# ELEKTRONN/ELEKTRONN2

Hardware: AMD Instinct MI355X
Metric: training_input_voxels_per_sec (higher is better)
Workload: dtype f32; 1 GPU; neuro3d_lite (1,1,23,183,183)->(1,2,10,37,37) fwd+bwd+Adam, 1 sample/GPU; parallelism=dp1, hipgraph=True, steps_per_launch=10

## Files before the change

elektronn2_amd/csrc/conv_first_mfma.hip:

```cpp
#include "common.hpp"
#include <algorithm>
#include <utility>

typedef float f32x4 __attribute__((ext_vector_type(4)));

template <class F, int... I>
__device__ __forceinline__ void fm_for_impl(F&& f, std::integer_sequence<int, I...>) {
  (f(std::integral_constant<int, I>{}), ...);
}
template <int N, class F>
__device__ __forceinline__ void fm_for(F&& f) {
  fm_for_impl(f, std::make_integer_sequence<int, N>{});
}
template <int ABID>
__device__ __forceinline__ f32x4 fm_mfma(float a, float b, f32x4 c) {
  return __builtin_amdgcn_mfma_f32_4x4x1f32(a, b, c, 4, ABID, 0);
}

namespace {

typedef __bf16 fm_bf16x8 __attribute__((ext_vector_type(8)));

struct FirstM {
  const float* x;
  const float* w;
  const float* bias;
  float* out;
  const float* dout;
  int N, Cout, D, H, W;
  int Ho, Wo;
  long xsN, xsD, xsH;
  long osN, osC, osD, osH;
  int act;
  int tilesX, tilesY, nTiles;
  int dbg;
  __bf16* nxb;
  int nxKG;
};

#ifdef E2_DEBUG_ENV
#define FM_DBG(p, bit) (((p).dbg & (bit)) != 0)
#else
#define FM_DBG(p, bit) false
#endif

constexpr int kTW = 72;

template <int KH, int KW, int PY, int PX, int MG>
struct Geo {
  static constexpr int T = KH * KW;
  static constexpr int TPV = 16 / MG;
  static constexpr int NAV = (T + TPV - 1) / TPV;
  static constexpr int RT = 4 * PY + KH - 1;
  static constexpr int CH = 4 * MG;
};

template <int KH, int KW, int PY, int PX, int MG>
__device__ __forceinline__ void load_weights(const FirstM& p, int lane,
                                             float (&aw)[Geo<KH, KW, PY, PX, MG>::NAV]) {
  using G = Geo<KH, KW, PY, PX, MG>;
  const int b = lane >> 2, i = lane & 3;
  const int slot = b / MG, g = b - slot * MG;
  const int ch = 4 * g + i;
#pragma unroll
  for (int v = 0; v < G::NAV; ++v) {
    const int tap = v * G::TPV + slot;
    aw[v] = (slot < G::TPV && tap < G::T && ch < p.Cout) ? p.w[ch * G::T + (G::T - 1 - tap)] : 0.f;
  }
}

template <int KH, int KW, int PY, int PX, int MG>
__device__ __forceinline__ void load_tile(const FirstM& p, int tile, float* xt, int& n, int& z,
                                          int& row0, int& col0) {
  using G = Geo<KH, KW, PY, PX, MG>;
  const int tx_ = tile % p.tilesX;
  int r = tile / p.tilesX;
  const int ty_ = r % p.tilesY; r /= p.tilesY;
  z = r % p.D;
  n = r / p.D;
  row0 = ty_ * 4 * PY;
  col0 = tx_ * 64;
  const float* src = p.x + (long)n * p.xsN + (long)z * p.xsD;
  for (int e = threadIdx.x; e < G::RT * kTW; e += 256) {
    const int i = e / kTW, j = e - i * kTW;
    const int y = row0 + i, xx = col0 + j;
    xt[e] = (y < p.H && xx < p.W && !FM_DBG(p, 1)) ? src[(long)y * p.xsH + xx] : 0.f;
  }
}

template <int KH, int KW, int PY, int PX, int MG>
__device__ __forceinline__ void conv_rows(const float* xw, int lane,
                                          const float (&aw)[Geo<KH, KW, PY, PX, MG>::NAV],
                                          f32x4 (&acc)[MG][PY]) {
  using G = Geo<KH, KW, PY, PX, MG>;
#pragma unroll
  for (int g = 0; g < MG; ++g)
#pragma unroll
    for (int nb = 0; nb < PY; ++nb) acc[g][nb] = (f32x4){0.f, 0.f, 0.f, 0.f};
  fm_for<PY + KH - 1>([&](auto rr_) {
    constexpr int rr = decltype(rr_)::value;
    float bx[KW];
#pragma unroll
    for (int tx = 0; tx < KW; ++tx) bx[tx] = xw[rr * kTW + lane + tx];
    fm_for<PY>([&](auto nb_) {
      constexpr int nb = decltype(nb_)::value;
      constexpr int ty = rr - nb;
      if constexpr (ty >= 0 && ty < KH) {
        fm_for<KW>([&](auto tx_) {
          constexpr int tx = decltype(tx_)::value;
          constexpr int tap = ty * KW + tx;
          fm_for<MG>([&](auto g_) {
            constexpr int g = decltype(g_)::value;
            acc[g][nb] = fm_mfma<(tap % G::TPV) * MG + g>(aw[tap / G::TPV], bx[tx], acc[g][nb]);
          });
        });
      }
    });
  });
}

template <int KH, int KW, int PY, int PX, int MG>
__global__ __launch_bounds__(256) void firstm_fwd_kernel(FirstM p) {
  using G = Geo<KH, KW, PY, PX, MG>;
  __shared__ float xt[G::RT * kTW];
  const int lane = threadIdx.x & 63, wave = threadIdx.x >> 6;
  float aw[G::NAV];
  load_weights<KH, KW, PY, PX, MG>(p, lane, aw);
  float bs[MG][4];
#pragma unroll
  for (int g = 0; g < MG; ++g)
#pragma unroll
    for (int r = 0; r < 4; ++r) bs[g][r] = (4 * g + r < p.Cout) ? p.bias[4 * g + r] : 0.f;
  for (int tile = blockIdx.x; tile < p.nTiles; tile += gridDim.x) {
    int n, z, row0, col0;
    __syncthreads();
    load_tile<KH, KW, PY, PX, MG>(p, tile, xt, n, z, row0, col0);
    __syncthreads();
    f32x4 acc[MG][PY];
    if (!FM_DBG(p, 2)) conv_rows<KH, KW, PY, PX, MG>(xt + wave * PY * kTW, lane, aw, acc);
    else {
#pragma unroll
      for (int g = 0; g < MG; ++g)
#pragma unroll
        for (int nb = 0; nb < PY; ++nb) acc[g][nb] = (f32x4){xt[lane], 0.f, 0.f, 0.f};
    }
    const int prow = row0 / PY + wave;
    const int pcol = (col0 + lane) / PX;
    const bool ok = prow < p.Ho && pcol < p.Wo && (lane % PX) == 0;
    float* ob = p.out + (long)n * p.osN + (long)z * p.osD + (long)prow * p.osH + pcol;
#pragma unroll
    for (int g = 0; g < MG; ++g)
#pragma unroll
      for (int r = 0; r < 4; ++r) {
        float m = acc[g][0][r];
        if constexpr (PY == 2) m = fmaxf(m, acc[g][1][r]);
        if constexpr (PX == 2) m = fmaxf(m, __shfl_xor(m, 1, 64));
        const int ch = 4 * g + r;
        float v = 0.f;
        if (ch < p.Cout) {
          v = m + bs[g][r];
          if (p.act == E2_ACT_RELU) v = fmaxf(v, 0.f);
          if (ok && !(FM_DBG(p, 4) && ch > 0)) ob[(long)ch * p.osC] = v;
        }
        acc[g][0][r] = v;
      }
    if (p.nxb && ok) {
      __bf16* nb = p.nxb + ((((long)n * p.D + z) * p.nxKG) * ((long)p.Ho * p.Wo) + (long)prow * p.Wo + pcol) * 8;
#pragma unroll
      for (int kg = 0; kg < (MG + 1) / 2; ++kg) {
        if (kg >= p.nxKG) continue;
        fm_bf16x8 h;
#pragma unroll
        for (int e = 0; e < 8; ++e) {
          const int g = 2 * kg + (e >> 2);
          h[e] = (__bf16)(g < MG ? acc[g < MG ? g : 0][0][e & 3] : 0.f);
        }
        *reinterpret_cast<fm_bf16x8*>(nb + (long)kg * p.Ho * p.Wo * 8) = h;
      }
    }
  }
}

template <int KH, int KW, int PY, int PX, int MG>
__global__ __launch_bounds__(256) void firstm_bwd_kernel(FirstM p, float* __restrict__ part) {
  using G = Geo<KH, KW, PY, PX, MG>;
  constexpr int T = G::T, CH = G::CH, NP = 64 * PY;
  constexpr bool Q4 = T <= 16;
  extern __shared__ __attribute__((aligned(16))) float fm_lds[];
  float* dyT = fm_lds;
  float* xt = fm_lds + 4 * NP * CH;
  const int lane = threadIdx.x & 63, wave = threadIdx.x >> 6;
  float aw[G::NAV];
  load_weights<KH, KW, PY, PX, MG>(p, lane, aw);
  const int pq = Q4 ? (lane >> 4) : 0;
  const int tapi = Q4 ? (lane & 15) : lane;
  const int tapl = tapi < T ? tapi : 0;
  const int tapoff = (tapl / KW) * kTW + (tapl % KW) + pq;
  f32x4 dwacc[MG];
  float db[MG][4];
#pragma unroll
  for (int g = 0; g < MG; ++g) {
    dwacc[g] = (f32x4){0.f, 0.f, 0.f, 0.f};
#pragma unroll
    for (int r = 0; r < 4; ++r) db[g][r] = 0.f;
  }
  float* dyw = dyT + wave * NP * CH;
  float bs[MG][4];
#pragma unroll
  for (int g = 0; g < MG; ++g)
#pragma unroll
    for (int r = 0; r < 4; ++r) bs[g][r] = (4 * g + r < p.Cout) ? p.bias[4 * g + r] : 0.f;
  for (int tile = blockIdx.x; tile < p.nTiles; tile += gridDim.x) {
    int n, z, row0, col0;
    __syncthreads();
    load_tile<KH, KW, PY, PX, MG>(p, tile, xt, n, z, row0, col0);
    const int prow = row0 / PY + wave;
    const int pcol = (col0 + lane) / PX;
    const bool ok = prow < p.Ho && pcol < p.Wo;
    const float* gp = p.dout + (long)n * p.osN + (long)z * p.osD + (long)prow * p.osH + pcol;
    float gvs[MG][4];
#pragma unroll
    for (int g = 0; g < MG; ++g)
#pragma unroll
      for (int r = 0; r < 4; ++r)
        gvs[g][r] = (ok && 4 * g + r < p.Cout) ? gp[(long)(4 * g + r) * p.osC] : 0.f;
    __syncthreads();
    const float* xw = xt + wave * PY * kTW;
    f32x4 acc[MG][PY];
    if (!FM_DBG(p, 2)) conv_rows<KH, KW, PY, PX, MG>(xw, lane, aw, acc);
    else {
#pragma unroll
      for (int g = 0; g < MG; ++g)
#pragma unroll
        for (int nb = 0; nb < PY; ++nb) acc[g][nb] = (f32x4){xw[lane], 0.f, 0.f, 0.f};
    }
#pragma unroll
    for (int g = 0; g < MG; ++g) {
#pragma unroll
      for (int r = 0; r < 4; ++r) {
        float m = acc[g][0][r];
        if constexpr (PY == 2) m = fmaxf(m, acc[g][1][r]);
        if constexpr (PX == 2) m = fmaxf(m, __shfl_xor(m, 1, 64));
        float gv = gvs[g][r];
        if (p.act == E2_ACT_RELU) {
          const float pre = m + bs[g][r];
          gv *= (pre > 0.f) ? 1.f : ((pre == 0.f) ? 0.5f : 0.f);
        }
        if ((lane % PX) == 0) db[g][r] += gv;
#pragma unroll
        for (int nb = 0; nb < PY; ++nb) acc[g][nb][r] = (acc[g][nb][r] == m) ? gv : 0.f;
      }
#pragma unroll
      for (int nb = 0; nb < PY; ++nb)
        *reinterpret_cast<f32x4*>(dyw + (nb * 64 + lane) * CH + 4 * g) = acc[g][nb];
    }
    const float* xb = xw + tapoff;
    if (FM_DBG(p, 4)) continue;
    if constexpr (Q4) {
      fm_for<NP / 4>([&](auto k_) {
        constexpr int p0 = 4 * decltype(k_)::value;
        const float bv = xb[(p0 / 64) * kTW + (p0 % 64)];
#pragma unroll
        for (int g = 0; g < MG; ++g) {
          const float av = dyw[(p0 + pq) * CH + 4 * g + (lane & 3)];
          dwacc[g] = __builtin_amdgcn_mfma_f32_4x4x1f32(av, bv, dwacc[g], 0, 0, 0);
        }
      });
    } else {
      fm_for<NP / 16>([&](auto pb_) {
        constexpr int pb = decltype(pb_)::value;
        float ad[MG];
#pragma unroll
        for (int g = 0; g < MG; ++g) ad[g] = dyw[(pb * 16 + (lane >> 2)) * CH + 4 * g + (lane & 3)];
        fm_for<16>([&](auto pp_) {
          constexpr int pp = decltype(pp_)::value;
          constexpr int pos = pb * 16 + pp;
          const float bv = xb[(pos / 64) * kTW + (pos % 64)];
#pragma unroll
          for (int g = 0; g < MG; ++g) dwacc[g] = fm_mfma<pp>(ad[g], bv, dwacc[g]);
        });
      });
    }
  }
  __syncthreads();
  float* red = fm_lds;
#pragma unroll
  for (int g = 0; g < MG; ++g)
#pragma unroll
    for (int r = 0; r < 4; ++r) {
      float v = dwacc[g][r];
      if constexpr (Q4) {
        v += __shfl_xor(v, 16, 64);
        v += __shfl_xor(v, 32, 64);
      }
      float sb = db[g][r];
#pragma unroll
      for (int o = 32; o > 0; o >>= 1) sb += __shfl_xor(sb, o, 64);
      float* rw = red + (wave * CH + 4 * g + r) * (T + 1);
      if (lane < T) rw[lane] = v;
      if (lane == 0) rw[T] = sb;
    }
  __syncthreads();
  float* ps = part + blockIdx.x;
  const long nS = gridDim.x;
  for (int e = threadIdx.x; e < p.Cout * (T + 1); e += 256)
    ps[e * nS] = (red[e] + red[CH * (T + 1) + e]) + (red[2 * CH * (T + 1) + e] + red[3 * CH * (T + 1) + e]);
}

template <int KH, int KW, int PY, int PX, int MG>
int launch_fwd(e2_ctx* ctx, const FirstM& p, int grid) {
  hipLaunchKernelGGL((firstm_fwd_kernel<KH, KW, PY, PX, MG>), dim3(grid), dim3(256), 0, ctx->stream, p);
  E2_CHECK_HIP(hipGetLastError());
  return 0;
}
template <int KH, int KW, int PY, int PX, int MG>
int launch_bwd(e2_ctx* ctx, const FirstM& p, int grid, float* part) {
  using G = Geo<KH, KW, PY, PX, MG>;
  const size_t lds = sizeof(float) * (4 * 64 * PY * G::CH + G::RT * kTW);
  static bool attr_done = false;
  if (!attr_done) {
    E2_CHECK_HIP(hipFuncSetAttribute(reinterpret_cast<const void*>(&firstm_bwd_kernel<KH, KW, PY, PX, MG>),
                                     hipFuncAttributeMaxDynamicSharedMemorySize, 160 * 1024));
    attr_done = true;
  }
  hipLaunchKernelGGL((firstm_bwd_kernel<KH, KW, PY, PX, MG>), dim3(grid), dim3(256), lds, ctx->stream, p, part);
  E2_CHECK_HIP(hipGetLastError());
  return 0;
}

}

int e2i_firstm_mg(int cout) { return cout <= 20 ? 5 : (cout <= 32 ? 8 : 0); }

int e2i_firstm_grid(const e2_ctx* ctx, long nTiles) {
  return (int)std::min<long>(nTiles, std::min<long>((long)ctx->num_cu * (e2_dbg_env("E2_FM_GRID") ? e2_dbg_env_int("E2_FM_GRID") : 3), 1024));
}

static void fill(FirstM& p, const e2_tensor5* x, const e2_tensor5* o, int cout, int py, int px) {
  p.x = x->ptr;
  p.N = x->n; p.Cout = cout; p.D = x->d; p.H = x->h; p.W = x->w;
  p.Ho = o->h; p.Wo = o->w;
  p.xsN = x->sn; p.xsD = x->sd; p.xsH = x->sh;
  p.osN = o->sn; p.osC = o->sc; p.osD = o->sd; p.osH = o->sh;
  p.dbg = e2_dbg_env_int("E2_FM_DBG");
  p.tilesX = e2_cdiv(o->w * px, 64);
  p.tilesY = e2_cdiv(o->h, 4);
  p.nTiles = p.N * p.D * p.tilesY * p.tilesX;
}

#define E2_FM_DISPATCH(FN, ...)                                                        \
  if (v == 1 && mg == 5) return FN<4, 4, 2, 2, 5>(__VA_ARGS__);                       \
  if (v == 1 && mg == 8) return FN<4, 4, 2, 2, 8>(__VA_ARGS__);                       \
  if (v == 2 && mg == 5) return FN<6, 6, 2, 2, 5>(__VA_ARGS__);                       \
  if (v == 2 && mg == 8) return FN<6, 6, 2, 2, 8>(__VA_ARGS__);                       \
  if (v == 3 && mg == 5) return FN<3, 3, 1, 1, 5>(__VA_ARGS__);                       \
  if (v == 3 && mg == 8) return FN<3, 3, 1, 1, 8>(__VA_ARGS__);

int e2i_firstm_fwd(e2_ctx* ctx, int v, const e2_tensor5* x, const float* w, const float* bias,
                   int cout, int py, int px, int act, const e2_tensor5* out, void* next_xb, int next_kg) {
  const int mg = e2i_firstm_mg(cout);
  FirstM p{};
  fill(p, x, out, cout, py, px);
  p.w = w; p.bias = bias; p.out = out->ptr; p.act = act;
  E2_REQUIRE(!next_xb || (next_kg * 8 >= cout && ((uintptr_t)next_xb & 15) == 0),
             "conv1(mfma): the next layer's copy holds %d channel groups for %d channels", next_kg, cout);
  p.nxb = reinterpret_cast<__bf16*>(next_xb); p.nxKG = next_kg;
  const int grid = e2i_firstm_grid(ctx, p.nTiles);
  E2_FM_DISPATCH(launch_fwd, ctx, p, grid)
  e2_set_error("conv1(mfma): no instance for variant %d, %d channels", v, cout);
  return 2;
}

size_t e2i_firstm_ws_floats(long nTiles, int cout, int T) {
  return (size_t)std::min<long>(nTiles, 1024) * cout * (T + 1);
}

int e2i_firstm_bwd(e2_ctx* ctx, int v, const e2_tensor5* x, const float* w, const float* bias,
                   const e2_tensor5* dout, int py, int px, int act, float* part, int* nslots) {
  const int cout = dout->c;
  const int mg = e2i_firstm_mg(cout);
  FirstM p{};
  fill(p, x, dout, cout, py, px);
  p.w = w; p.bias = bias; p.dout = dout->ptr; p.act = act;
  const int grid = e2i_firstm_grid(ctx, p.nTiles);
  *nslots = grid;
  E2_FM_DISPATCH(launch_bwd, ctx, p, grid, part)
  e2_set_error("conv1(mfma): no instance for variant %d, %d channels", v, cout);
  return 2;
}
```

Measured before the change: 521.9 million voxels/s.

## Trim index math and loads in first-layer MFMA conv kernels

Replaces the per-tile integer div/mod tile decode with precomputed magic-number division and switches strides to 32-bit unsigned offsets, checked on the host. The tile load is restructured from a strided loop into unrolled per-wave row loads with a separate halo load. The max-pool neighbour exchange uses DPP instead of a shuffle, and the epilogue is specialised for relu and full-channel cases. The backward pass folds the activation test into an infinite bias when there is no relu. The aim is to cut scalar and vector integer overhead in a small, latency-bound first layer, at the cost of more code and range checks that reject large tensors.

```diff
diff --git a/elektronn2_amd/csrc/conv_first_mfma.hip b/elektronn2_amd/csrc/conv_first_mfma.hip
--- a/elektronn2_amd/csrc/conv_first_mfma.hip
+++ b/elektronn2_amd/csrc/conv_first_mfma.hip
@@ -17,9 +17,31 @@
   return __builtin_amdgcn_mfma_f32_4x4x1f32(a, b, c, 4, ABID, 0);
 }
 
+__device__ __forceinline__ float fm_xor1(float v) {
+  return __int_as_float(__builtin_amdgcn_mov_dpp(__float_as_int(v), 0xB1, 0xF, 0xF, true));
+}
+
+__device__ __forceinline__ int fm_per_tile(int v) {
+  asm volatile("" : "+s"(v));
+  return v;
+}
+
 namespace {
 
 typedef __bf16 fm_bf16x8 __attribute__((ext_vector_type(8)));
+
+struct FmDiv { unsigned m, sh; };
+inline FmDiv fm_mk_div(unsigned d) {
+  unsigned l = 0;
+  while ((1ull << l) < d) ++l;
+  FmDiv f;
+  f.m = (unsigned)(((1ull << (31 + l)) + d - 1) / d);
+  f.sh = l;
+  return f;
+}
+__device__ __forceinline__ unsigned fm_div(unsigned n, const FmDiv& f) {
+  return __umulhi(2u * n + 1u, f.m) >> f.sh;
+}
 
 struct FirstM {
   const float* x;
@@ -29,10 +51,11 @@
   const float* dout;
   int N, Cout, D, H, W;
   int Ho, Wo;
-  long xsN, xsD, xsH;
-  long osN, osC, osD, osH;
+  unsigned xsN, xsD, xsH;
+  unsigned osN, osC, osD, osH;
   int act;
   int tilesX, tilesY, nTiles;
+  FmDiv dX, dY, dD;
   int dbg;
   __bf16* nxb;
   int nxKG;
@@ -52,6 +75,7 @@
   static constexpr int TPV = 16 / MG;
   static constexpr int NAV = (T + TPV - 1) / TPV;
   static constexpr int RT = 4 * PY + KH - 1;
+  static constexpr int RTL = (RT + 7) / 8 * 8;
   static constexpr int CH = 4 * MG;
 };
 
@@ -69,23 +93,39 @@
   }
 }
 
-template <int KH, int KW, int PY, int PX, int MG>
-__device__ __forceinline__ void load_tile(const FirstM& p, int tile, float* xt, int& n, int& z,
-                                          int& row0, int& col0) {
-  using G = Geo<KH, KW, PY, PX, MG>;
-  const int tx_ = tile % p.tilesX;
-  int r = tile / p.tilesX;
-  const int ty_ = r % p.tilesY; r /= p.tilesY;
-  z = r % p.D;
-  n = r / p.D;
-  row0 = ty_ * 4 * PY;
-  col0 = tx_ * 64;
-  const float* src = p.x + (long)n * p.xsN + (long)z * p.xsD;
-  for (int e = threadIdx.x; e < G::RT * kTW; e += 256) {
-    const int i = e / kTW, j = e - i * kTW;
-    const int y = row0 + i, xx = col0 + j;
-    xt[e] = (y < p.H && xx < p.W && !FM_DBG(p, 1)) ? src[(long)y * p.xsH + xx] : 0.f;
-  }
+template <int PY>
+__device__ __forceinline__ void decode_tile(const FirstM& p, int tile, int& n, int& z, int& row0, int& col0) {
+  const unsigned r1 = fm_div((unsigned)tile, p.dX), tx_ = (unsigned)tile - r1 * (unsigned)p.tilesX;
+  const unsigned r2 = fm_div(r1, p.dY), ty_ = r1 - r2 * (unsigned)p.tilesY;
+  const unsigned n_ = fm_div(r2, p.dD);
+  n = (int)n_;
+  z = (int)(r2 - n_ * (unsigned)p.D);
+  row0 = (int)ty_ * 4 * PY;
+  col0 = (int)tx_ * 64;
+}
+
+template <int KH, int KW, int PY, int PX, int MG>
+__device__ __forceinline__ void load_tile(const FirstM& p, float* xt, int lane, int wave, int n, int z,
+                                          int row0, int col0) {
+  using G = Geo<KH, KW, PY, PX, MG>;
+  const float* src = p.x + (unsigned long)n * p.xsN + (unsigned long)z * p.xsD +
+                     (unsigned long)row0 * p.xsH + col0;
+  const int hrem = p.H - row0, wrem = p.W - col0;
+  float v[G::RTL / 4 + 1];
+  bool in[G::RTL / 4 + 1];
+#pragma unroll
+  for (int k = 0; k < G::RTL / 4; ++k) {
+    const int i = wave + 4 * k;
+    in[k] = i < hrem && lane < wrem && !FM_DBG(p, 1);
+    v[k] = src[in[k] ? (unsigned)i * p.xsH + (unsigned)lane : 0u];
+  }
+  const int hi = 4 * wave + (lane >> 3), hj = 64 + (lane & 7);
+  const bool halo = lane < 32 && hi < G::RTL;
+  in[G::RTL / 4] = halo && hi < hrem && hj < wrem && !FM_DBG(p, 1);
+  v[G::RTL / 4] = src[in[G::RTL / 4] ? (unsigned)hi * p.xsH + (unsigned)hj : 0u];
+#pragma unroll
+  for (int k = 0; k < G::RTL / 4; ++k) xt[(wave + 4 * k) * kTW + lane] = in[k] ? v[k] : 0.f;
+  if (halo) xt[hi * kTW + hj] = in[G::RTL / 4] ? v[G::RTL / 4] : 0.f;
 }
 
 template <int KH, int KW, int PY, int PX, int MG>
@@ -120,10 +160,10 @@
 }
 
 template <int KH, int KW, int PY, int PX, int MG>
-__global__ __launch_bounds__(256) void firstm_fwd_kernel(FirstM p) {
-  using G = Geo<KH, KW, PY, PX, MG>;
-  __shared__ float xt[G::RT * kTW];
-  const int lane = threadIdx.x & 63, wave = threadIdx.x >> 6;
+__global__ __launch_bounds__(256, 3) void firstm_fwd_kernel(FirstM p) {
+  using G = Geo<KH, KW, PY, PX, MG>;
+  __shared__ float xt[G::RTL * kTW];
+  const int lane = threadIdx.x & 63, wave = __builtin_amdgcn_readfirstlane(threadIdx.x >> 6);
   float aw[G::NAV];
   load_weights<KH, KW, PY, PX, MG>(p, lane, aw);
   float bs[MG][4];
@@ -131,10 +171,13 @@
   for (int g = 0; g < MG; ++g)
 #pragma unroll
     for (int r = 0; r < 4; ++r) bs[g][r] = (4 * g + r < p.Cout) ? p.bias[4 * g + r] : 0.f;
+  const bool relu = p.act == E2_ACT_RELU, full = p.Cout == G::CH;
+  const unsigned cstep = p.osC * 4u;
   for (int tile = blockIdx.x; tile < p.nTiles; tile += gridDim.x) {
     int n, z, row0, col0;
+    decode_tile<PY>(p, tile, n, z, row0, col0);
     __syncthreads();
-    load_tile<KH, KW, PY, PX, MG>(p, tile, xt, n, z, row0, col0);
+    load_tile<KH, KW, PY, PX, MG>(p, xt, lane, wave, n, z, row0, col0);
     __syncthreads();
     f32x4 acc[MG][PY];
     if (!FM_DBG(p, 2)) conv_rows<KH, KW, PY, PX, MG>(xt + wave * PY * kTW, lane, aw, acc);
@@ -147,35 +190,64 @@
     const int prow = row0 / PY + wave;
     const int pcol = (col0 + lane) / PX;
     const bool ok = prow < p.Ho && pcol < p.Wo && (lane % PX) == 0;
-    float* ob = p.out + (long)n * p.osN + (long)z * p.osD + (long)prow * p.osH + pcol;
 #pragma unroll
     for (int g = 0; g < MG; ++g)
 #pragma unroll
       for (int r = 0; r < 4; ++r) {
         float m = acc[g][0][r];
         if constexpr (PY == 2) m = fmaxf(m, acc[g][1][r]);
-        if constexpr (PX == 2) m = fmaxf(m, __shfl_xor(m, 1, 64));
-        const int ch = 4 * g + r;
-        float v = 0.f;
-        if (ch < p.Cout) {
-          v = m + bs[g][r];
-          if (p.act == E2_ACT_RELU) v = fmaxf(v, 0.f);
-          if (ok && !(FM_DBG(p, 4) && ch > 0)) ob[(long)ch * p.osC] = v;
+        if constexpr (PX == 2) m = fmaxf(m, fm_xor1(m));
+        acc[g][0][r] = m;
+      }
+    auto epilogue = [&](auto relu_, auto full_) {
+      constexpr bool RELU = decltype(relu_)::value, FULL = decltype(full_)::value;
+      const int cout = FULL ? G::CH : fm_per_tile(p.Cout);
+#pragma unroll
+      for (int g = 0; g < MG; ++g)
+#pragma unroll
+        for (int r = 0; r < 4; ++r) {
+          float v = 0.f;
+          if (FULL || 4 * g + r < cout) {
+            v = acc[g][0][r] + bs[g][r];
+            if constexpr (RELU) v = fmaxf(v, 0.f);
+          }
+          acc[g][0][r] = v;
         }
-        acc[g][0][r] = v;
-      }
-    if (p.nxb && ok) {
-      __bf16* nb = p.nxb + ((((long)n * p.D + z) * p.nxKG) * ((long)p.Ho * p.Wo) + (long)prow * p.Wo + pcol) * 8;
-#pragma unroll
-      for (int kg = 0; kg < (MG + 1) / 2; ++kg) {
-        if (kg >= p.nxKG) continue;
-        fm_bf16x8 h;
-#pragma unroll
-        for (int e = 0; e < 8; ++e) {
-          const int g = 2 * kg + (e >> 2);
-          h[e] = (__bf16)(g < MG ? acc[g < MG ? g : 0][0][e & 3] : 0.f);
+      if (ok) {
+        char* ob = reinterpret_cast<char*>(p.out + (unsigned long)n * p.osN + (unsigned long)z * p.osD);
+        unsigned vo = ((unsigned)prow * p.osH + (unsigned)pcol) * 4u;
+#pragma unroll
+        for (int g = 0; g < MG; ++g)
+#pragma unroll
+          for (int r = 0; r < 4; ++r) {
+            const int ch = 4 * g + r;
+            if ((FULL || ch < cout) && !(FM_DBG(p, 4) && ch > 0)) *reinterpret_cast<float*>(ob + vo) = acc[g][0][r];
+            vo += cstep;
+          }
+      }
+    };
+    if (relu) {
+      if (full) epilogue(std::true_type{}, std::true_type{});
+      else epilogue(std::true_type{}, std::false_type{});
+    } else {
+      if (full) epilogue(std::false_type{}, std::true_type{});
+      else epilogue(std::false_type{}, std::false_type{});
+    }
+    if (p.nxb) {
+      const int nkg = fm_per_tile(p.nxKG);
+      __bf16* nb = p.nxb + ((((long)n * p.D + z) * nkg) * ((long)p.Ho * p.Wo) + (long)prow * p.Wo + pcol) * 8;
+      if (ok) {
+#pragma unroll
+        for (int kg = 0; kg < (MG + 1) / 2; ++kg) {
+          if (kg >= nkg) continue;
+          fm_bf16x8 h;
+#pragma unroll
+          for (int e = 0; e < 8; ++e) {
+            const int g = 2 * kg + (e >> 2);
+            h[e] = (__bf16)(g < MG ? acc[g < MG ? g : 0][0][e & 3] : 0.f);
+          }
+          *reinterpret_cast<fm_bf16x8*>(nb + (long)kg * p.Ho * p.Wo * 8) = h;
         }
-        *reinterpret_cast<fm_bf16x8*>(nb + (long)kg * p.Ho * p.Wo * 8) = h;
       }
     }
   }
@@ -189,7 +261,7 @@
   extern __shared__ __attribute__((aligned(16))) float fm_lds[];
   float* dyT = fm_lds;
   float* xt = fm_lds + 4 * NP * CH;
-  const int lane = threadIdx.x & 63, wave = threadIdx.x >> 6;
+  const int lane = threadIdx.x & 63, wave = __builtin_amdgcn_readfirstlane(threadIdx.x >> 6);
   float aw[G::NAV];
   load_weights<KH, KW, PY, PX, MG>(p, lane, aw);
   const int pq = Q4 ? (lane >> 4) : 0;
@@ -210,20 +282,49 @@
   for (int g = 0; g < MG; ++g)
 #pragma unroll
     for (int r = 0; r < 4; ++r) bs[g][r] = (4 * g + r < p.Cout) ? p.bias[4 * g + r] : 0.f;
+  if (p.act != E2_ACT_RELU) {
+#pragma unroll
+    for (int g = 0; g < MG; ++g)
+#pragma unroll
+      for (int r = 0; r < 4; ++r) bs[g][r] = __builtin_inff();
+  }
+  const bool full = p.Cout == CH;
+  const unsigned cstep = p.osC * 4u;
   for (int tile = blockIdx.x; tile < p.nTiles; tile += gridDim.x) {
     int n, z, row0, col0;
+    decode_tile<PY>(p, tile, n, z, row0, col0);
     __syncthreads();
-    load_tile<KH, KW, PY, PX, MG>(p, tile, xt, n, z, row0, col0);
+    load_tile<KH, KW, PY, PX, MG>(p, xt, lane, wave, n, z, row0, col0);
     const int prow = row0 / PY + wave;
     const int pcol = (col0 + lane) / PX;
     const bool ok = prow < p.Ho && pcol < p.Wo;
-    const float* gp = p.dout + (long)n * p.osN + (long)z * p.osD + (long)prow * p.osH + pcol;
     float gvs[MG][4];
 #pragma unroll
     for (int g = 0; g < MG; ++g)
 #pragma unroll
-      for (int r = 0; r < 4; ++r)
-        gvs[g][r] = (ok && 4 * g + r < p.Cout) ? gp[(long)(4 * g + r) * p.osC] : 0.f;
+      for (int r = 0; r < 4; ++r) gvs[g][r] = 0.f;
+    if (ok) {
+      const char* gb = reinterpret_cast<const char*>(p.dout + (unsigned long)n * p.osN + (unsigned long)z * p.osD);
+      unsigned vo = ((unsigned)prow * p.osH + (unsigned)pcol) * 4u;
+      if (full) {
+#pragma unroll
+        for (int g = 0; g < MG; ++g)
+#pragma unroll
+          for (int r = 0; r < 4; ++r) {
+            gvs[g][r] = *reinterpret_cast<const float*>(gb + vo);
+            vo += cstep;
+          }
+      } else {
+        const int cout = fm_per_tile(p.Cout);
+#pragma unroll
+        for (int g = 0; g < MG; ++g)
+#pragma unroll
+          for (int r = 0; r < 4; ++r) {
+            if (4 * g + r < cout) gvs[g][r] = *reinterpret_cast<const float*>(gb + vo);
+            vo += cstep;
+          }
+      }
+    }
     __syncthreads();
     const float* xw = xt + wave * PY * kTW;
     f32x4 acc[MG][PY];
@@ -240,13 +341,11 @@
       for (int r = 0; r < 4; ++r) {
         float m = acc[g][0][r];
         if constexpr (PY == 2) m = fmaxf(m, acc[g][1][r]);
-        if constexpr (PX == 2) m = fmaxf(m, __shfl_xor(m, 1, 64));
+        if constexpr (PX == 2) m = fmaxf(m, fm_xor1(m));
         float gv = gvs[g][r];
-        if (p.act == E2_ACT_RELU) {
-          const float pre = m + bs[g][r];
-          gv *= (pre > 0.f) ? 1.f : ((pre == 0.f) ? 0.5f : 0.f);
-        }
-        if ((lane % PX) == 0) db[g][r] += gv;
+        const float pre = m + bs[g][r];
+        gv *= (pre > 0.f) ? 1.f : ((pre == 0.f) ? 0.5f : 0.f);
+        db[g][r] += gv;
 #pragma unroll
         for (int nb = 0; nb < PY; ++nb) acc[g][nb][r] = (acc[g][nb][r] == m) ? gv : 0.f;
       }
@@ -293,7 +392,7 @@
         v += __shfl_xor(v, 16, 64);
         v += __shfl_xor(v, 32, 64);
       }
-      float sb = db[g][r];
+      float sb = (lane % PX) == 0 ? db[g][r] : 0.f;
 #pragma unroll
       for (int o = 32; o > 0; o >>= 1) sb += __shfl_xor(sb, o, 64);
       float* rw = red + (wave * CH + 4 * g + r) * (T + 1);
@@ -316,7 +415,7 @@
 template <int KH, int KW, int PY, int PX, int MG>
 int launch_bwd(e2_ctx* ctx, const FirstM& p, int grid, float* part) {
   using G = Geo<KH, KW, PY, PX, MG>;
-  const size_t lds = sizeof(float) * (4 * 64 * PY * G::CH + G::RT * kTW);
+  const size_t lds = sizeof(float) * (4 * 64 * PY * G::CH + G::RTL * kTW);
   static bool attr_done = false;
   if (!attr_done) {
     E2_CHECK_HIP(hipFuncSetAttribute(reinterpret_cast<const void*>(&firstm_bwd_kernel<KH, KW, PY, PX, MG>),
@@ -336,16 +435,26 @@
   return (int)std::min<long>(nTiles, std::min<long>((long)ctx->num_cu * (e2_dbg_env("E2_FM_GRID") ? e2_dbg_env_int("E2_FM_GRID") : 3), 1024));
 }
 
-static void fill(FirstM& p, const e2_tensor5* x, const e2_tensor5* o, int cout, int py, int px) {
+static int fill(FirstM& p, const e2_tensor5* x, const e2_tensor5* o, int cout, int py, int px) {
+  const long lim = 1L << 31;
+  E2_REQUIRE(x->sn >= 0 && x->sn < lim && x->sd >= 0 && x->sd < lim && x->sh >= 0 && x->sh < (1L << 24) &&
+                 o->sn >= 0 && o->sn < lim && o->sd >= 0 && o->sd < lim && o->sh >= 0 && o->sc >= 0 &&
+                 (long)(cout - 1) * o->sc + (long)o->h * o->sh + o->w < (1L << 30),
+             "conv1(mfma): strides (%ld,%ld,%ld) / (%ld,%ld,%ld,%ld) are out of the 32-bit offset range",
+             (long)x->sn, (long)x->sd, (long)x->sh, (long)o->sn, (long)o->sc, (long)o->sd, (long)o->sh);
   p.x = x->ptr;
   p.N = x->n; p.Cout = cout; p.D = x->d; p.H = x->h; p.W = x->w;
   p.Ho = o->h; p.Wo = o->w;
-  p.xsN = x->sn; p.xsD = x->sd; p.xsH = x->sh;
-  p.osN = o->sn; p.osC = o->sc; p.osD = o->sd; p.osH = o->sh;
+  p.xsN = (unsigned)x->sn; p.xsD = (unsigned)x->sd; p.xsH = (unsigned)x->sh;
+  p.osN = (unsigned)o->sn; p.osC = (unsigned)o->sc; p.osD = (unsigned)o->sd; p.osH = (unsigned)o->sh;
   p.dbg = e2_dbg_env_int("E2_FM_DBG");
   p.tilesX = e2_cdiv(o->w * px, 64);
   p.tilesY = e2_cdiv(o->h, 4);
-  p.nTiles = p.N * p.D * p.tilesY * p.tilesX;
+  const long nTiles = (long)p.N * p.D * p.tilesY * p.tilesX;
+  E2_REQUIRE(nTiles < (1L << 30), "conv1(mfma): %ld tiles", nTiles);
+  p.nTiles = (int)nTiles;
+  p.dX = fm_mk_div(p.tilesX); p.dY = fm_mk_div(p.tilesY); p.dD = fm_mk_div(p.D);
+  return 0;
 }
 
 #define E2_FM_DISPATCH(FN, ...)                                                        \
@@ -360,7 +469,7 @@
                    int cout, int py, int px, int act, const e2_tensor5* out, void* next_xb, int next_kg) {
   const int mg = e2i_firstm_mg(cout);
   FirstM p{};
-  fill(p, x, out, cout, py, px);
+  if (int rc = fill(p, x, out, cout, py, px)) return rc;
   p.w = w; p.bias = bias; p.out = out->ptr; p.act = act;
   E2_REQUIRE(!next_xb || (next_kg * 8 >= cout && ((uintptr_t)next_xb & 15) == 0),
              "conv1(mfma): the next layer's copy holds %d channel groups for %d channels", next_kg, cout);
@@ -380,7 +489,7 @@
   const int cout = dout->c;
   const int mg = e2i_firstm_mg(cout);
   FirstM p{};
-  fill(p, x, dout, cout, py, px);
+  if (int rc = fill(p, x, dout, cout, py, px)) return rc;
   p.w = w; p.bias = bias; p.dout = dout->ptr; p.act = act;
   const int grid = e2i_firstm_grid(ctx, p.nTiles);
   *nslots = grid;
```

Measured after the change: 525.1 million voxels/s, median of 6. About the same (+0.6%).
